# CX9898/sddmm-gpu

Measured on AMD Instinct MI355X. Metric: SDDMM GFLOP/s (2·nnz·K) + HBM GB/s %peak, K=128, 1/2/4/8 MI355X, higher is better.
Workload: dtype f32

## Files before the change

sddmm-gpu_amd/csrc/sddmm.hip:

```cpp
#include <algorithm>
#include <type_traits>
#include <cmath>
#include <vector>

#include "common.hpp"
#include "plan.hpp"

namespace bsmr {
namespace {

typedef float f32x4 __attribute__((ext_vector_type(4)));

struct SddmmArgs {
    const float* A;
    const float* B;
    float* P;
    u32 d0, nd;
    const u32* tileRows;
    const u32* rows;
    u32 R, N, K;
    const u32* denseCols;
    const u32* blockValues;
    const uint2* slots;
    u32 nslots;
// ... 302 lines not shown
}

struct RbArgs {
    const char* A;
    const char* B;
    float* P;
    const u32* rows;
    u32 R, N, RB;
    u32 qbase;
    u32 row0;
    const uint4* items;
    const u32* itemEnd;
    const uint2* pieces;
    const u32* meta;
    const u32* out;
    const uint4* tilePanel;
    const u32* tileIds;
    const u32* denseCols;
    const u32* blockValues;
    u32 mode;
    u32 outLds;
    u32 outPacked;
    u32 stageNt;
    u32 lateB;
    u32 stageBlocks;
    const u32* sortedPos;
    const uint2* itemEnt;
    const uint2* runs;
    const uint2* itemRuns;
    u32 pairs;
    unsigned long long* trace;
    u32 diag;
    unsigned long long bA, bB, bP;
};

typedef float f32x2 __attribute__((ext_vector_type(2)));
typedef _Float16 h16x2 __attribute__((ext_vector_type(2)));
typedef __bf16 b16x2 __attribute__((ext_vector_type(2)));
typedef _Float16 h16x8 __attribute__((ext_vector_type(8)));
typedef __bf16 b16x8 __attribute__((ext_vector_type(8)));

template <int DT>
__device__ __forceinline__ u32 lds_chunk(u32 lr, u32 c) {
    if constexpr (DT == 0)
        return c;
    else
        return (c & ~3u) | ((c & 3u) ^ (lr & 3u));
}

__device__ __forceinline__ f32x4 ld16(const char* p) { return *reinterpret_cast<const f32x4*>(p); }

__device__ __forceinline__ u32 lds_addr(const char* l) {
    return __builtin_amdgcn_readfirstlane(static_cast<u32>(
        reinterpret_cast<uintptr_t>((__attribute__((address_space(3))) const char*)l)));
}
template <int AUX>
__device__ __forceinline__ void rb_dma16(const char* g, const u32 m0) {
    if constexpr (AUX == 2)
        asm volatile("s_mov_b32 m0, %1\n\ts_nop 0\n\tglobal_load_lds_dwordx4 %0, off nt" ::"v"(g), "s"(m0)
                     : "memory", "m0");
    else
        asm volatile("s_mov_b32 m0, %1\n\ts_nop 0\n\tglobal_load_lds_dwordx4 %0, off" ::"v"(g), "s"(m0)
                     : "memory", "m0");
}

template <int I>
__device__ __forceinline__ u32 quad_bcast(u32 v) {
    return static_cast<u32>(
        __builtin_amdgcn_update_dpp(0, static_cast<int>(v), I * 0x55, 0xF, 0xF, false));
}

template <int DT>
__device__ __forceinline__ void chunk_dot(const f32x4 a, const f32x4 b, f32x2& acc0, f32x2& acc1) {
    if constexpr (DT == 0) {
        acc0 = __builtin_elementwise_fma(f32x2{a.x, a.y}, f32x2{b.x, b.y}, acc0);
        acc1 = __builtin_elementwise_fma(f32x2{a.z, a.w}, f32x2{b.z, b.w}, acc1);
    } else if constexpr (DT == 1) {
        const h16x8 ha = __builtin_bit_cast(h16x8, a), hb = __builtin_bit_cast(h16x8, b);
        acc0.x = __builtin_amdgcn_fdot2(ha.s01, hb.s01, acc0.x, false);
        acc0.y = __builtin_amdgcn_fdot2(ha.s23, hb.s23, acc0.y, false);
        acc1.x = __builtin_amdgcn_fdot2(ha.s45, hb.s45, acc1.x, false);
        acc1.y = __builtin_amdgcn_fdot2(ha.s67, hb.s67, acc1.y, false);
    } else {
        const b16x8 ha = __builtin_bit_cast(b16x8, a), hb = __builtin_bit_cast(b16x8, b);
        acc0.x = __builtin_amdgcn_fdot2_f32_bf16(ha.s01, hb.s01, acc0.x, false);
        acc0.y = __builtin_amdgcn_fdot2_f32_bf16(ha.s23, hb.s23, acc0.y, false);
        acc1.x = __builtin_amdgcn_fdot2_f32_bf16(ha.s45, hb.s45, acc1.x, false);
        acc1.y = __builtin_amdgcn_fdot2_f32_bf16(ha.s67, hb.s67, acc1.y, false);
    }
}

template <int DT>
__device__ __forceinline__ f32x4 chunk_mfma(const f32x4 a, const f32x4 b, f32x4 acc) {
    if constexpr (DT == 0) {
        acc = __builtin_amdgcn_mfma_f32_16x16x4f32(a.x, b.x, acc, 0, 0, 0);
        acc = __builtin_amdgcn_mfma_f32_16x16x4f32(a.y, b.y, acc, 0, 0, 0);
        acc = __builtin_amdgcn_mfma_f32_16x16x4f32(a.z, b.z, acc, 0, 0, 0);
        return __builtin_amdgcn_mfma_f32_16x16x4f32(a.w, b.w, acc, 0, 0, 0);
    } else if constexpr (DT == 1) {
        return __builtin_amdgcn_mfma_f32_16x16x32_f16(__builtin_bit_cast(h16x8, a),
                                                      __builtin_bit_cast(h16x8, b), acc, 0, 0, 0);
    } else {
        return __builtin_amdgcn_mfma_f32_16x16x32_bf16(__builtin_bit_cast(b16x8, a),
                                                       __builtin_bit_cast(b16x8, b), acc, 0, 0, 0);
    }
}

template <int RBY>
struct RowGeom {
    static constexpr u32 G = RBY >= 2048 ? 16 : RBY >= 1024 ? 8 : 4;
    static constexpr u32 NC = RBY / (16 * G);
    static constexpr u32 NB = (RB_PIECE_MAX + G - 1) / G;
    static constexpr u32 RR = (G == 4 ? 4u : G == 8 ? 2u : 1u) < NC ? (G == 4 ? 4u : G == 8 ? 2u : 1u) : NC;
};

template <int G, int I>
__device__ __forceinline__ u32 group_bcast(u32 v) {
    if constexpr (G == 4)
        return quad_bcast<I>(v);
    else if constexpr (G == 8)
        return static_cast<u32>(__builtin_amdgcn_ds_swizzle(static_cast<int>(v), 0x18 | (I << 5)));
    else
        return row_bcast<I>(v);
}

template <int DT, int RBY>
struct DenseTileLds {
    static constexpr int NK = RBY / 64;
    static constexpr int CH = NK > 8 ? 8 : NK;
    u32 lr, c, idx[4];
    __device__ __forceinline__ static u32 chunk(int kk, u32 g) {
        if constexpr (NK >= 4)
            return 16 * (kk >> 2) + 4 * g + (kk & 3);
        else
            return NK * g + kk;
    }
    __device__ __forceinline__ void meta(const RbArgs& a, const u32 tile, const u32 q0) {
        const u32 l = __lane_id(), rr = l & 15, g = l >> 4;
        const u32 p = a.tilePanel[tile].x;
        c = a.denseCols[tile * 16 + rr];
        const u32* bvals = a.blockValues + static_cast<size_t>(tile) * 256 + 64 * g + rr;
#pragma unroll
        for (int r = 0; r < 4; ++r) idx[r] = bvals[16 * r];
        lr = p * 16 - q0 + rr;
    }
    __device__ __forceinline__ void loadB(const RbArgs& a, const int k0, f32x4 (&bv)[CH]) const {
        const u32 g = __lane_id() >> 4;
        const bool cvalid = c < a.N;
        const char* bcol = a.B + static_cast<size_t>(cvalid && !(a.diag & 8388608u) ? c : 0) * RBY;
#pragma unroll
        for (int kk = 0; kk < CH; ++kk)
            bv[kk] = cvalid ? ld16(bcol + 16 * chunk(k0 + kk, g)) : f32x4{0, 0, 0, 0};
    }
    __device__ __forceinline__ void load(const RbArgs& a, const u32 tile, const u32 q0,
                                         f32x4 (&bv)[CH]) {
        meta(a, tile, q0);
        loadB(a, 0, bv);
    }
    __device__ __forceinline__ void run(const RbArgs& a, const char* As, f32x4 (&bv)[CH]) const {
        const u32 g = __lane_id() >> 4;
        const char* arow = As + lr * RBY;
        f32x4 acc0 = {0, 0, 0, 0}, acc1 = {0, 0, 0, 0};
#pragma unroll
        for (int k0 = 0; k0 < NK; k0 += CH) {
            if (k0) loadB(a, k0, bv);
#pragma unroll
            for (int kk = 0; kk < CH; ++kk) {
                const f32x4 av = ld16(arow + 16 * lds_chunk<DT>(lr, chunk(k0 + kk, g)));
                f32x4& acc = (kk & 1) ? acc1 : acc0;
                acc = chunk_mfma<DT>(av, bv[kk], acc);
            }
        }
        const f32x4 acc = acc0 + acc1;
#pragma unroll
        for (int r = 0; r < 4; ++r)
            if (idx[r] != NULLV) a.P[idx[r]] = acc[r];
    }
};

template <int RBY>
__device__ __forceinline__ void load_bcol(const RbArgs& a, const u32 col, const u32 sub,
                                          const u32 (&rot)[RowGeom<RBY>::NC],
                                          f32x4 (&bv)[RowGeom<RBY>::NC]) {
    const u32 bb = ((a.diag & 64) ? 0u : col) * RBY + 16 * sub;
#pragma unroll
    for (u32 f = 0; f < RowGeom<RBY>::NC; ++f)
        bv[f] = f + RowGeom<RBY>::RR <= RowGeom<RBY>::NC
                    ? ld16(a.B + (bb + rot[0]) + 16 * RowGeom<RBY>::G * f)
                    : ld16(a.B + (bb + rot[f]));
}

template <int RBY>
struct Piece {
    u32 first, len, col;
    u32 mm[RowGeom<RBY>::NB], mo[RowGeom<RBY>::NB];
};

template <int RBY>
__device__ __forceinline__ void load_piece_desc(const RbArgs& a, const u32 pi, Piece<RBY>& pc) {
    const uint2 d = a.pieces[pi];
    pc.first = d.x;
    pc.len = (d.y >> 22) + 1;
    pc.col = d.y & 0x3FFFFFu;
}

template <int RBY>
__device__ __forceinline__ void load_piece_body(const RbArgs& a, const u32 sub,
                                                const u32 (&rot)[RowGeom<RBY>::NC],
                                                f32x4 (&bv)[RowGeom<RBY>::NC], Piece<RBY>& pc) {
    constexpr u32 G = RowGeom<RBY>::G;
    load_bcol<RBY>(a, pc.col, sub, rot, bv);
#pragma unroll
    for (u32 k = 0; k < RowGeom<RBY>::NB; ++k) {
        const u32 e = G * k + sub;
        pc.mm[k] = e < pc.len ? a.meta[pc.first + e] : 0u;
        pc.mo[k] = !a.outLds && !a.outPacked && e < pc.len ? a.out[pc.first + e] : 0u;
    }
}

template <int RBY>
__device__ __forceinline__ void load_piece(const RbArgs& a, const u32 pi, const u32 sub,
                                           const u32 (&rot)[RowGeom<RBY>::NC],
                                           f32x4 (&bv)[RowGeom<RBY>::NC], Piece<RBY>& pc) {
    load_piece_desc<RBY>(a, pi, pc);
    load_piece_body<RBY>(a, sub, rot, bv, pc);
}

template <int DT, int RBY>
__device__ __forceinline__ void residual_piece(const RbArgs& a, const char* As,
                                               const Piece<RBY>& pc, const u32 sub,
                                               const u32 (&rot)[RowGeom<RBY>::NC],
                                               const f32x4 (&bv)[RowGeom<RBY>::NC]) {
    constexpr u32 G = RowGeom<RBY>::G, NC = RowGeom<RBY>::NC;
#pragma unroll
    for (u32 k = 0; k < RowGeom<RBY>::NB; ++k) {
        if (G * k >= pc.len) break;
        const u32 nb = min(G, pc.len - G * k);
        const u32 mk = DT == 0 ? (pc.mm[k] >> 22) * RBY : pc.mm[k];
        float res = 0.f;
#pragma unroll
        for (int i = 0; i < static_cast<int>(G); ++i) {
            if (static_cast<u32>(i) >= nb) break;
            u32 m;
            switch (i) {
#define BSMR_C(I) \
    case I: m = group_bcast<G, (I < G ? I : 0)>(mk); break;
                BSMR_C(0) BSMR_C(1) BSMR_C(2) BSMR_C(3) BSMR_C(4) BSMR_C(5) BSMR_C(6) BSMR_C(7)
                BSMR_C(8) BSMR_C(9) BSMR_C(10) BSMR_C(11) BSMR_C(12) BSMR_C(13) BSMR_C(14)
#undef BSMR_C
                default: m = group_bcast<G, G - 1>(mk); break;
            }
            u32 ab;
            if constexpr (DT == 0) {
                ab = m + 16 * sub;
            } else {
                const u32 lr = m >> 22;
                ab = lr * RBY + 16 * lds_chunk<DT>(lr, sub);
            }
            const char* arot = As + (ab + rot[0]);
            f32x2 acc0 = {0.f, 0.f}, acc1 = {0.f, 0.f};
            constexpr u32 H = NC > 4 ? NC / 2 : NC;
#pragma unroll
            for (u32 h = 0; h < NC; h += H) {
                f32x4 av[H];
#pragma unroll
                for (u32 f = 0; f < H; ++f)
                    av[f] = h + f + RowGeom<RBY>::RR <= NC ? ld16(arot + 16 * G * (h + f))
                                                           : ld16(As + (ab + rot[h + f]));
#pragma unroll
                for (u32 f = 0; f < H; ++f) {
                    if constexpr (DT == 0)
                        chunk_dot<DT>(av[f], bv[h + f], acc0, acc0);
                    else
                        chunk_dot<DT>(av[f], bv[h + f], acc0, acc1);
                }
            }
            f32x2 acc = acc0;
            if constexpr (DT != 0) acc += acc1;
            float sm = acc.x + acc.y;
            sm += dppf<0xB1>(sm);
            sm += dppf<0x4E>(sm);
            if constexpr (G >= 8) sm += dppf<0x141>(sm);
            if constexpr (G == 16) sm += dppf<0x140>(sm);
            if (sub == static_cast<u32>(i)) res = sm;
        }
        if (sub < nb) {
            if (a.outLds)
                *reinterpret_cast<float*>(const_cast<char*>(As) + a.outLds +
                                          4 * (pc.mm[k] & 0x3FFFFFu)) = res;
            else
                a.P[a.outPacked ? pc.mm[k] & 0x3FFFFFu : pc.mo[k]] = res;
        }
    }
}

constexpr u32 BATCH_CTR_BYTES = 16;
template <int DT, int RBY, int NT, typename LoadRuns>
__device__ __forceinline__ void rb_batches(const RbArgs& a, const char* As, const u32 p0, const u32 np,
                                           const u32 gr, const u32 sub, const u32 (&rot)[RowGeom<RBY>::NC],
                                           Piece<RBY>& pc, f32x4 (&pre)[RowGeom<RBY>::NC], LoadRuns&& load_runs) {
    constexpr u32 NC = RowGeom<RBY>::NC, GW = 64 / RowGeom<RBY>::G, NW = NT / 64;
    u32* const ctr = reinterpret_cast<u32*>(const_cast<char*>(As) + (NT == 1024 ? 160u : 80u) * 1024u - 4u);
    auto grab = [&]() -> u32 {
        u32 v = 0;
        if ((threadIdx.x & 63) == 0)
            v = __hip_atomic_fetch_add(ctr, 1u, __ATOMIC_RELAXED, __HIP_MEMORY_SCOPE_WORKGROUP);
        return NW + static_cast<u32>(__builtin_amdgcn_readfirstlane(static_cast<int>(v)));
    };
    Piece<RBY> pn;
    f32x4 nb[NC];
    auto fetch = [&](const u32 b) {
        const u32 pi = b * GW + gr % GW;
        pn.len = 0;
        if (pi < np) load_piece<RBY>(a, p0 + pi, sub, rot, nb, pn);
    };
    u32 bn = grab();
    if (bn * GW < np)
        fetch(bn);
    else
        load_runs();
    if (pc.len) residual_piece<DT, RBY>(a, As, pc, sub, rot, pre);
    while (bn * GW < np) {
        pc = pn;
#pragma unroll
        for (u32 f = 0; f < NC; ++f) pre[f] = nb[f];
        bn = grab();
        if (bn * GW < np)
            fetch(bn);
        else
            load_runs();
        if (pc.len) residual_piece<DT, RBY>(a, As, pc, sub, rot, pre);
    }
}

constexpr u32 NO_ITEM = 0xFFFFFFFFu;
constexpr u32 PAIR_RUNS_PER_WAVE = 16;

template <int RBY, int NT>
__device__ __forceinline__ u32 rb_stage_rows(const RbArgs& a, const u32 q0, const u32 ws, const u32 lane) {
    constexpr u32 NW = NT / 64, NCH = RBY / 16, NR = NCH >= 64 ? 1 : 64 / NCH;
    constexpr u32 MAXB = (NT == 1024 ? 160u : 80u) / NW;
    const u32 i = lane / NR, b = ws + i * NW, lr = 64 * b / NCH + lane % NR, q = q0 + lr;
    return (i < MAXB && lr < a.RB && q < a.R) ? a.rows[q] : a.row0;
}

template <int DT, int RBY, int NT, int AUX>
__device__ __forceinline__ void rb_stage_issue(const RbArgs& a, char* As, u32 rowv, const u32 ws,
                                               const u32 lane) {
    constexpr u32 NW = NT / 64, NCH = RBY / 16, NR = NCH >= 64 ? 1 : 64 / NCH;
    asm volatile("" : "+v"(rowv));
    constexpr u32 MAXB = (NT == 1024 ? 160u : 80u) / NW;
    const u32 x0 = 64 * ws + lane;
    const u32 coff = 16 * lds_chunk<DT>(x0 / NCH, x0 % NCH);
#pragma unroll 2
    for (u32 i = 0; i < MAXB; ++i) {
        const u32 b = ws + i * NW;
        u32 src = static_cast<u32>(__builtin_amdgcn_readlane(static_cast<int>(rowv), i * NR));
#pragma unroll
        for (u32 k = 1; k < NR; ++k) {
            const u32 rk = static_cast<u32>(__builtin_amdgcn_readlane(static_cast<int>(rowv), i * NR + k));
            src = lane / NCH == k ? rk : src;
        }
        const char* g = a.A + (static_cast<size_t>(src) * RBY + coff);
        if (b < a.stageBlocks) rb_dma16<AUX>(g, lds_addr(As) + 1024 * b);
    }
}

template <int DT, int RBY, int NT, int OM, bool DYN = false>
__device__ __forceinline__ bool rb_item(const RbArgs& a, char* As, const u32 idx, const bool prestaged,
                                        const u32 next) {
    constexpr bool PAIR = OM == 2, STAGED = OM != 0, LEAN = OM >= 2;
    using Geo = RowGeom<RBY>;
    constexpr u32 G = Geo::G, NC = Geo::NC;
    constexpr u32 NW = NT / 64;
    constexpr u32 NG = NT / G;
    constexpr u32 TC = DenseTileLds<DT, RBY>::CH;
    const unsigned long long t0 = LEAN ? 0ull : rtime(a.trace);
    uint4 it = a.items[idx];
    it.x = __builtin_amdgcn_readfirstlane(it.x);
    it.y = __builtin_amdgcn_readfirstlane(it.y);
    it.z = __builtin_amdgcn_readfirstlane(it.z);
    it.w = __builtin_amdgcn_readfirstlane(it.w);
    const u32 pend = a.itemEnd[idx];
    if (it.y == it.z && it.w == pend) return false;
    bool has_next = false, same_rb = false;
    u32 q0n = 0;
    if (next != NO_ITEM) {
        uint4 nt = a.items[next];
        nt.x = __builtin_amdgcn_readfirstlane(nt.x);
        nt.y = __builtin_amdgcn_readfirstlane(nt.y);
        nt.z = __builtin_amdgcn_readfirstlane(nt.z);
        nt.w = __builtin_amdgcn_readfirstlane(nt.w);
        const u32 nend = __builtin_amdgcn_readfirstlane(a.itemEnd[next]);
        has_next = !(nt.y == nt.z && nt.w == nend);
        q0n = a.qbase + nt.x * a.RB;
        same_rb = nt.x == it.x;
    }
    const u32 q0 = a.qbase + it.x * a.RB;
    u32 tid = threadIdx.x;
    if constexpr (LEAN) asm volatile("" : "+v"(tid));
    const u32 w = tid >> 6, sub = tid % G, j = (tid & 63) / G;
    const u32 ntile = !LEAN && (a.mode & 1) ? it.z - it.y : 0u;
    const u32 np = (a.mode & 2) ? pend - it.w : 0u;
    const u32 gr = tid / G;
    u32 rot[NC];
#pragma unroll
    for (u32 f = 0; f < NC; ++f) rot[f] = 16u * G * ((f + j % Geo::RR) % NC);
    constexpr u32 NCH = RBY / 16;
    constexpr u32 NR = NCH >= 64 ? 1 : 64 / NCH;
    constexpr u32 MAXB = (NT == 1024 ? 160u : 80u) / NW;
    static_assert(MAXB * NW == (NT == 1024 ? 160u : 80u), "whole KiB blocks");
    constexpr bool ROWV = MAXB * NR <= 64;
    const u32 lane = tid & 63;
    const u32 ws = __builtin_amdgcn_readfirstlane(w);
    u32 rowv = 0;
    u32 src[ROWV ? 1 : MAXB];
    if (!prestaged) {
        if constexpr (ROWV) {
            rowv = rb_stage_rows<RBY, NT>(a, q0, ws, lane);
        } else {
#pragma unroll
            for (u32 i = 0; i < MAXB; ++i) {
                const u32 lr = 64 * (ws + i * NW) / NCH + lane / NCH, q = q0 + lr;
                src[i] = lr < a.RB && q < a.R ? a.rows[q] : a.row0;
            }
#pragma unroll
            for (u32 i = 0; i < MAXB; ++i) asm volatile("" : "+v"(src[i]));
        }
    }
    f32x4 tb[TC], pre[NC];
    DenseTileLds<DT, RBY> dt;
    const u32 tw = NW - 1 - w;
    Piece<RBY> pc;
    pc.len = 0;
    if constexpr (!LEAN)
        if (tw < ntile) dt.meta(a, a.tileIds[it.y + tw], q0);
    if (gr < np) load_piece_desc<RBY>(a, it.w + gr, pc);
    uint2 myrun = make_uint2(0u, 0u), irun = make_uint2(0u, 0u);
    u32 rown = a.row0;
    auto load_runs = [&]() {
        if (STAGED && a.runs && a.outLds) {
            irun = a.itemRuns[idx];
            irun.x = __builtin_amdgcn_readfirstlane(irun.x);
            irun.y = __builtin_amdgcn_readfirstlane(irun.y);
            const u32 jr = w + NW * lane;
            if (jr < irun.y) myrun = a.runs[irun.x + jr];
        }
        if constexpr (ROWV)
            if (has_next && !same_rb) rown = rb_stage_rows<RBY, NT>(a, q0n, ws, lane);
    };
    auto stage = [&](auto aux_tag) {
        constexpr int AUX = decltype(aux_tag)::value;
        if constexpr (ROWV) {
            rb_stage_issue<DT, RBY, NT, AUX>(a, As, rowv, ws, lane);
        } else {
            const u32 x0 = 64 * ws + lane;
            const u32 coff = 16 * lds_chunk<DT>(x0 / NCH, x0 % NCH);
#pragma unroll
            for (u32 i = 0; i < MAXB; ++i) {
                const u32 b = ws + i * NW;
                const char* g = a.A + (static_cast<size_t>(src[i]) * RBY + coff);
                if (b < a.stageBlocks) rb_dma16<AUX>(g, lds_addr(As) + 1024 * b);
            }
        }
    };
    if (!prestaged) {
        if (!LEAN && a.stageNt)
            stage(std::integral_constant<int, 2>{});
        else
            stage(std::integral_constant<int, 0>{});
    }
    if (!LEAN && !a.lateB) {
        if (gr < np) load_piece_body<RBY>(a, sub, rot, pre, pc);
        if (tw < ntile) dt.loadB(a, 0, tb);
    }
    if constexpr (DYN)
        if (tid == 0) *reinterpret_cast<u32*>(As + (NT == 1024 ? 160u : 80u) * 1024u - 4u) = 0u;
    asm volatile("s_waitcnt vmcnt(0)" ::: "memory");
    __syncthreads();
    if (LEAN || a.lateB) {
        if (gr < np) load_piece_body<RBY>(a, sub, rot, pre, pc);
        if constexpr (!LEAN)
            if (tw < ntile) dt.loadB(a, 0, tb);
    }
    const unsigned long long tm = LEAN ? 0ull : rtime(a.trace);
    if (!LEAN && (a.diag & 8)) {
        trace_wave(a.trace, idx * NW + w, t0, tm);
        return false;
    }
    if constexpr (!LEAN)
        if (tw < ntile) dt.run(a, As, tb);
    const unsigned long long td = LEAN ? 0ull : rtime(a.trace);
    if constexpr (DYN) {
        rb_batches<DT, RBY, NT>(a, As, it.w, np, gr, sub, rot, pc, pre, [] {});
    } else {
        Piece<RBY> pn;
        f32x4 nb[NC];
        auto fetch = [&](const u32 ph) {
            const u32 pi = ph * NG + ((ph & 1) ? NG - 1 - gr : gr);
            pn.len = 0;
            if (pi < np) load_piece<RBY>(a, it.w + pi, sub, rot, nb, pn);
        };
        if (NG < np) fetch(1);
        if (pc.len) residual_piece<DT, RBY>(a, As, pc, sub, rot, pre);
        for (u32 ph = 1; ph * NG < np; ++ph) {
            pc = pn;
#pragma unroll
            for (u32 f = 0; f < NC; ++f) pre[f] = nb[f];
            if ((ph + 1) * NG < np) fetch(ph + 1);
            if (pc.len) residual_piece<DT, RBY>(a, As, pc, sub, rot, pre);
        }
    }
    if constexpr (STAGED) load_runs();
    if constexpr (!LEAN) {
        for (u32 t = it.y + tw + NW; t < it.z; t += NW) {
            dt.load(a, a.tileIds[t], q0, tb);
            dt.run(a, As, tb);
        }
    }
    bool staged_next = false;
    if (STAGED && a.outLds) {
        __syncthreads();
        const uint2 ie = a.itemEnt[idx];
        const float* res = reinterpret_cast<const float*>(As + a.outLds);
        const u32 nr = irun.y > w ? (irun.y - w + NW - 1) / NW : 0u;
        if constexpr (PAIR && ROWV) {
            if (has_next && __builtin_amdgcn_readfirstlane(irun.y) <= NW * PAIR_RUNS_PER_WAVE) {
                float v[PAIR_RUNS_PER_WAVE];
#pragma unroll
                for (u32 u = 0; u < PAIR_RUNS_PER_WAVE; ++u) {
                    const u32 sl = static_cast<u32>(__builtin_amdgcn_readlane(static_cast<int>(myrun.y), u));
                    const u32 len = u < nr ? sl >> 16 : 0u;
                    v[u] = lane < len ? res[(sl & 0xFFFFu) + lane] : 0.0f;
                }
                __syncthreads();
                rowv = rown;
                if (!same_rb) stage(std::integral_constant<int, 0>{});
#pragma unroll
                for (u32 u = 0; u < PAIR_RUNS_PER_WAVE; ++u) {
                    const u32 pos = static_cast<u32>(__builtin_amdgcn_readlane(static_cast<int>(myrun.x), u));
                    const u32 sl = static_cast<u32>(__builtin_amdgcn_readlane(static_cast<int>(myrun.y), u));
                    const u32 len = u < nr ? sl >> 16 : 0u;
                    if (lane < len) a.P[pos + lane] = v[u];
                }
                return true;
            }
        }
        if (LEAN || !(a.diag & 128)) {
            if (LEAN || a.runs) {
                for (u32 i = 0; i < nr; i += 4) {
                    u32 pos[4], s0[4], len[4];
                    float v[4];
#pragma unroll
                    for (u32 u = 0; u < 4; ++u) {
                        const u32 q = min(i + u, 63u);
                        pos[u] = static_cast<u32>(__builtin_amdgcn_readlane(static_cast<int>(myrun.x), q));
                        const u32 sl = static_cast<u32>(__builtin_amdgcn_readlane(static_cast<int>(myrun.y), q));
                        s0[u] = sl & 0xFFFFu;
                        len[u] = i + u < nr ? sl >> 16 : 0u;
                        v[u] = lane < len[u] ? res[s0[u] + lane] : 0.0f;
                    }
#pragma unroll
                    for (u32 u = 0; u < 4; ++u)
                        if (lane < len[u]) a.P[pos[u] + lane] = v[u];
                }
            } else if constexpr (!LEAN) {
                constexpr u32 U = 8;
                for (u32 t0s = tid; t0s < ie.y; t0s += U * NT) {
                    u32 pos[U];
#pragma unroll
                    for (u32 k = 0; k < U; ++k) {
                        const u32 t = t0s + k * NT;
                        pos[k] = t < ie.y ? a.sortedPos[ie.x + t] : 0u;
                    }
#pragma unroll
                    for (u32 k = 0; k < U; ++k) {
                        const u32 t = t0s + k * NT;
                        if (t < ie.y) a.P[pos[k]] = res[t];
                    }
                }
            }
        }
        if constexpr (PAIR && ROWV) {
            if (has_next) {
                __syncthreads();
                rowv = rown;
                if (!same_rb) stage(std::integral_constant<int, 0>{});
                staged_next = true;
            }
        }
    }
    if constexpr (!LEAN) trace_wave(a.trace, idx * NW + w, t0, tm, td);
    return staged_next;
}

template <int DT, int RBY, int NT, bool DYN, bool LITE = false>
__global__ __launch_bounds__(NT, 4) void k_sddmm_rb(RbArgs a) {
    extern __shared__ __attribute__((aligned(16))) char AsB[];
    char* As = AsB;
    if (blockIdx.y) {
        a.A += blockIdx.y * a.bA;
        a.B += blockIdx.y * a.bB;
        a.P += blockIdx.y * a.bP;
    }
    using Geo = RowGeom<RBY>;
    constexpr u32 G = Geo::G, NC = Geo::NC;
    constexpr u32 NW = NT / 64;
    constexpr u32 NG = NT / G;
    constexpr u32 TC = DenseTileLds<DT, RBY>::CH;
    const unsigned long long t0 = LITE ? 0ull : rtime(a.trace);
    uint4 it = a.items[blockIdx.x];
    it.x = __builtin_amdgcn_readfirstlane(it.x);
    it.y = __builtin_amdgcn_readfirstlane(it.y);
    it.z = __builtin_amdgcn_readfirstlane(it.z);
    it.w = __builtin_amdgcn_readfirstlane(it.w);
    const u32 pend = a.itemEnd[blockIdx.x];
    if (it.y == it.z && it.w == pend) return;
    const u32 q0 = a.qbase + it.x * a.RB;
    const u32 tid = threadIdx.x, w = tid >> 6, sub = tid % G, j = (tid & 63) / G;
    const u32 ntile = !LITE && (a.mode & 1) ? it.z - it.y : 0u;
    const u32 np = LITE || (a.mode & 2) ? pend - it.w : 0u;
    const u32 gr = tid / G;
    u32 rot[NC];
#pragma unroll
    for (u32 f = 0; f < NC; ++f) rot[f] = 16u * G * ((f + j % Geo::RR) % NC);
    constexpr u32 NCH = RBY / 16;
    constexpr u32 NR = NCH >= 64 ? 1 : 64 / NCH;
    constexpr u32 MAXB = (NT == 1024 ? 160u : 80u) / NW;
    static_assert(MAXB * NW == (NT == 1024 ? 160u : 80u), "whole KiB blocks");
    constexpr bool ROWV = MAXB * NR <= 64;
    const u32 lane = tid & 63;
    const u32 ws = __builtin_amdgcn_readfirstlane(w);
    u32 rowv = a.row0;
    u32 src[ROWV ? 1 : MAXB];
    if constexpr (ROWV) {
        const u32 i = lane / NR, b = ws + i * NW, lr = 64 * b / NCH + lane % NR, q = q0 + lr;
        if (i < MAXB && lr < a.RB && q < a.R) rowv = a.rows[q];
    } else {
#pragma unroll
        for (u32 i = 0; i < MAXB; ++i) {
            const u32 lr = 64 * (ws + i * NW) / NCH + lane / NCH, q = q0 + lr;
            src[i] = lr < a.RB && q < a.R ? a.rows[q] : a.row0;
        }
#pragma unroll
        for (u32 i = 0; i < MAXB; ++i) asm volatile("" : "+v"(src[i]));
    }
    f32x4 tb[TC], pre[NC];
    DenseTileLds<DT, RBY> dt;
    const u32 tw = NW - 1 - w;
    Piece<RBY> pc;
    pc.len = 0;
    if constexpr (!LITE)
        if (tw < ntile) dt.meta(a, a.tileIds[it.y + tw], q0);
    if (gr < np) load_piece_desc<RBY>(a, it.w + gr, pc);
    uint2 myrun = make_uint2(0u, 0u), irun = make_uint2(0u, 0u);
    auto load_runs = [&]() {
        if (!LITE && a.runs && a.outLds) {
            irun = a.itemRuns[blockIdx.x];
            irun.x = __builtin_amdgcn_readfirstlane(irun.x);
            irun.y = __builtin_amdgcn_readfirstlane(irun.y);
            const u32 j = w + NW * lane;
            if (j < irun.y) myrun = a.runs[irun.x + j];
        }
    };
    auto stage = [&](auto aux_tag) {
        constexpr int AUX = decltype(aux_tag)::value;
        const u32 x0 = 64 * ws + lane;
        const u32 coff = 16 * lds_chunk<DT>(x0 / NCH, x0 % NCH);
        if constexpr (ROWV) {
#pragma unroll
            for (u32 i = 0; i < MAXB; ++i) {
                const u32 b = ws + i * NW;
                u32 src = static_cast<u32>(__builtin_amdgcn_readlane(static_cast<int>(rowv), i * NR));
#pragma unroll
                for (u32 k = 1; k < NR; ++k) {
                    const u32 rk = static_cast<u32>(__builtin_amdgcn_readlane(static_cast<int>(rowv), i * NR + k));
                    src = lane / NCH == k ? rk : src;
                }
                const char* g = a.A + (static_cast<size_t>(src) * RBY + coff);
                if (b < a.stageBlocks) rb_dma16<AUX>(g, lds_addr(As) + 1024 * b);
            }
        } else {
#pragma unroll
            for (u32 i = 0; i < MAXB; ++i) {
                const u32 b = ws + i * NW;
                const char* g = a.A + (static_cast<size_t>(src[i]) * RBY + coff);
                if (b < a.stageBlocks) rb_dma16<AUX>(g, lds_addr(As) + 1024 * b);
            }
        }
    };
    if (!LITE && a.stageNt)
        stage(std::integral_constant<int, 2>{});
    else
        stage(std::integral_constant<int, 0>{});
    if (!LITE && !a.lateB) {
        if (gr < np) load_piece_body<RBY>(a, sub, rot, pre, pc);
        if (tw < ntile) dt.loadB(a, 0, tb);
    }
    if constexpr (DYN)
        if (tid == 0) *reinterpret_cast<u32*>(As + (NT == 1024 ? 160u : 80u) * 1024u - 4u) = 0u;
    asm volatile("s_waitcnt vmcnt(0)" ::: "memory");
    __syncthreads();
    if (LITE || a.lateB) {
        if (gr < np) load_piece_body<RBY>(a, sub, rot, pre, pc);
        if constexpr (!LITE)
            if (tw < ntile) dt.loadB(a, 0, tb);
    }
    const unsigned long long tm = LITE ? 0ull : rtime(a.trace);
    if (!LITE && (a.diag & 8)) {
        trace_wave(a.trace, blockIdx.x * NW + w, t0, tm);
        return;
    }
    if constexpr (!LITE)
        if (tw < ntile) dt.run(a, As, tb);
    const unsigned long long td = LITE ? 0ull : rtime(a.trace);
    if constexpr (DYN) {
        rb_batches<DT, RBY, NT>(a, As, it.w, np, gr, sub, rot, pc, pre, load_runs);
    } else {
        Piece<RBY> pn;
        f32x4 nb[NC];
        auto fetch = [&](const u32 ph) {
            const u32 pi = ph * NG + ((ph & 1) ? NG - 1 - gr : gr);
            pn.len = 0;
            if (pi < np) load_piece<RBY>(a, it.w + pi, sub, rot, nb, pn);
        };
        if (NG < np)
            fetch(1);
        else
            load_runs();
        if (pc.len) residual_piece<DT, RBY>(a, As, pc, sub, rot, pre);
        for (u32 ph = 1; ph * NG < np; ++ph) {
            pc = pn;
#pragma unroll
            for (u32 f = 0; f < NC; ++f) pre[f] = nb[f];
            if ((ph + 1) * NG < np)
                fetch(ph + 1);
            else
                load_runs();
            if (pc.len) residual_piece<DT, RBY>(a, As, pc, sub, rot, pre);
        }
    }
    if constexpr (LITE) return;
    for (u32 t = it.y + tw + NW; t < it.z; t += NW) {
        dt.load(a, a.tileIds[t], q0, tb);
        dt.run(a, As, tb);
    }
    if (a.outLds) {
        __syncthreads();
        const uint2 ie = a.itemEnt[blockIdx.x];
        const float* res = reinterpret_cast<const float*>(As + a.outLds);
        if (!(a.diag & 128)) {
            constexpr u32 U = 8;
            auto pass = [&]() {
                for (u32 t0 = tid; t0 < ie.y; t0 += U * NT) {
                    u32 pos[U];
#pragma unroll
                    for (u32 k = 0; k < U; ++k) {
                        const u32 t = t0 + k * NT;
                        pos[k] = t < ie.y ? a.sortedPos[ie.x + t] : 0u;
                    }
#pragma unroll
                    for (u32 k = 0; k < U; ++k) {
                        const u32 t = t0 + k * NT;
                        if (t < ie.y) a.P[pos[k]] = res[t];
                    }
                }
            };
            if (a.runs) {
                const u32 nr = irun.y > w ? (irun.y - w + NW - 1) / NW : 0u;
                for (u32 i = 0; i < nr; i += 4) {
                    u32 pos[4], s0[4], len[4];
                    float v[4];
#pragma unroll
                    for (u32 u = 0; u < 4; ++u) {
                        const u32 q = min(i + u, 63u);
                        pos[u] = static_cast<u32>(__builtin_amdgcn_readlane(static_cast<int>(myrun.x), q));
                        const u32 sl = static_cast<u32>(__builtin_amdgcn_readlane(static_cast<int>(myrun.y), q));
                        s0[u] = sl & 0xFFFFu;
                        len[u] = i + u < nr ? sl >> 16 : 0u;
                        v[u] = lane < len[u] ? res[s0[u] + lane] : 0.0f;
                    }
#pragma unroll
                    for (u32 u = 0; u < 4; ++u)
                        if (lane < len[u]) a.P[pos[u] + lane] = v[u];
                }
            } else {
                pass();
            }
        }
    }
    trace_wave(a.trace, blockIdx.x * NW + w, t0, tm, td);
}

template <int DT, int RBY, int NT, bool DYN>
__global__ __launch_bounds__(NT, 4) void k_sddmm_rb_pair(RbArgs a) {
    extern __shared__ __attribute__((aligned(16))) char AsB[];
    char* As = AsB;
    if (blockIdx.y) {
        a.A += blockIdx.y * a.bA;
        a.B += blockIdx.y * a.bB;
        a.P += blockIdx.y * a.bP;
    }
    const u32 x = blockIdx.x % XCD_BUCKETS, i0 = (blockIdx.x / XCD_BUCKETS) * 2 * XCD_BUCKETS + x;
    if (rb_item<DT, RBY, NT, 2, DYN>(a, As, i0, false, i0 + XCD_BUCKETS))
        rb_item<DT, RBY, NT, 2, DYN>(a, As, i0 + XCD_BUCKETS, true, NO_ITEM);
}

template <int DT, int RBY>
void (*pick_rb(const u32 NT, const bool pairs, const bool dyn, const bool lite))(RbArgs) {
    if constexpr (RBY >= 256) {
        if (pairs) {
            if constexpr (RBY <= 512)
                if (dyn) return NT == 1024 ? k_sddmm_rb_pair<DT, RBY, 1024, true> : k_sddmm_rb_pair<DT, RBY, 512, true>;
            return NT == 1024 ? k_sddmm_rb_pair<DT, RBY, 1024, false> : k_sddmm_rb_pair<DT, RBY, 512, false>;
        }
    }
    if constexpr (RBY <= 512)
        if (dyn) {
            if (lite) return NT == 1024 ? k_sddmm_rb<DT, RBY, 1024, true, true> : k_sddmm_rb<DT, RBY, 512, true, true>;
            return NT == 1024 ? k_sddmm_rb<DT, RBY, 1024, true> : k_sddmm_rb<DT, RBY, 512, true>;
        }
    if (lite) return NT == 1024 ? k_sddmm_rb<DT, RBY, 1024, false, true> : k_sddmm_rb<DT, RBY, 512, false, true>;
    return NT == 1024 ? k_sddmm_rb<DT, RBY, 1024, false> : k_sddmm_rb<DT, RBY, 512, false>;
}

static_assert(TILES_PER_ITEM == 1, "dense work items are single tiles (tile id = item id)");

using KernelFn = void (*)(SddmmArgs);

template <int G, bool PANELS>
KernelFn pick_k(u32 K) {
#define BSMR_K(KT) (PANELS ? k_sddmm_panels_f32<KT, G> : k_sddmm_f32<KT, G>)
    switch (K) {
        case 32: return BSMR_K(32);
        case 64: return BSMR_K(64);
        case 128: return BSMR_K(128);
        case 256: return BSMR_K(256);
        case 512: return BSMR_K(512);
        default: return BSMR_K(0);
    }
#undef BSMR_K
}

template <bool PANELS>
KernelFn pick_kernel(u32 K) {
    if (K % 64 == 0) return pick_k<16, PANELS>(K);
    if (K % 32 == 0) return pick_k<8, PANELS>(K);
    return pick_k<4, PANELS>(K);
}

int validate(const void* dA, const void* dB, u32 K, int dtype, const float* dP) {
    if (!dA || !dB || !dP) {
        set_error("bsmr_sddmm: null device pointer");
        return BSMR_ERR_INVALID;
    }
    return report(validate_kd("bsmr_sddmm", K, dtype));
}

SddmmArgs make_args(const Plan& p, const void* dA, const void* dB, u32 K, float* dP) {
    SddmmArgs a{};
    a.A = static_cast<const float*>(dA);
    a.B = static_cast<const float*>(dB);
    a.P = dP;
    a.tileRows = p.tileRows.data();
    a.rows = p.rows.data();
    a.R = p.R;
    a.N = p.N;
    a.K = K;
    a.denseCols = p.denseCols.data();
    a.blockValues = p.blockValues.data();
    a.slots = p.cmSlots.data();
    a.cmRow = p.cmRow.data();
    a.cmCol = p.cmCol.data();
    a.cmOut = p.cmOut.data();
    a.ritems = p.resItems.data();
    a.sparseValues = p.sparseValues.data();
    a.sparseRel = p.sparseRel.data();
    a.sparseCol = p.sparseColIdx.data();
    a.diag = p.diag;
    return a;
}

int get_rb_layout(const Plan& p, int slot, int dtype, u32 pa, u32 pb,
                  std::shared_ptr<const Plan::RowBlockLayout>* out, const LaunchSite* at = nullptr,
                  bool keep = false) {
    std::lock_guard<std::mutex> g(p.layout_mu);
    const u32 rowBytes = 128u << slot;
    const bool half = dtype != BSMR_F32;
    if (!keep) {
        *out = p.rowblock_ready(rowBytes, half, pa, pb);
        if (*out) return BSMR_OK;
        if (at) BSMR_CHECK(lazy_build_guard(*at));
    }
    int err = BSMR_OK;
// ... 462 lines not shown
```

Measured before the change: 20600.

## Software-pipeline piece descriptor loads two stages ahead with branchless clamped fetches

Restructures the residual-piece loop so descriptors are prefetched two iterations ahead (d1/d2), while bodies (meta, out, B columns) are loaded one ahead. Per-lane conditional loads are replaced by clamped index loads, and loop trip counts become wave-uniform via a per-wave activity check. This is meant to hide the dependent descriptor-to-body load latency and remove divergent branches. In exchange it issues redundant clamped loads for inactive lanes and adds register pressure from the extra in-flight descriptors.

Result: faster. 21060 (median of 6 runs) (+2.2%).

```diff
diff --git a/sddmm-gpu_amd/csrc/sddmm.hip b/sddmm-gpu_amd/csrc/sddmm.hip
--- a/sddmm-gpu_amd/csrc/sddmm.hip
+++ b/sddmm-gpu_amd/csrc/sddmm.hip
@@ -522,34 +522,30 @@
     u32 mm[RowGeom<RBY>::NB], mo[RowGeom<RBY>::NB];
 };
 
+
+__device__ __forceinline__ uint2 load_piece_desc(const RbArgs& a, const u32 p0, const u32 np, const u32 pi) {
+    return a.pieces[p0 + min(pi, np - 1u)];
+}
+
 template <int RBY>
-__device__ __forceinline__ void load_piece_desc(const RbArgs& a, const u32 pi, Piece<RBY>& pc) {
-    const uint2 d = a.pieces[pi];
-    pc.first = d.x;
-    pc.len = (d.y >> 22) + 1;
-    pc.col = d.y & 0x3FFFFFu;
-}
-
-template <int RBY>
-__device__ __forceinline__ void load_piece_body(const RbArgs& a, const u32 sub,
+__device__ __forceinline__ void load_piece_body(const RbArgs& a, const uint2 d, const bool has,
+                                                const bool use_out, const u32 sub,
                                                 const u32 (&rot)[RowGeom<RBY>::NC],
                                                 f32x4 (&bv)[RowGeom<RBY>::NC], Piece<RBY>& pc) {
-    constexpr u32 G = RowGeom<RBY>::G;
+    constexpr u32 G = RowGeom<RBY>::G, NB = RowGeom<RBY>::NB;
+    const u32 last = d.y >> 22;
+    pc.first = d.x;
+    pc.len = has ? last + 1u : 0u;
+    pc.col = d.y & 0x3FFFFFu;
+#pragma unroll
+    for (u32 k = 0; k < NB; ++k) pc.mo[k] = 0u;
+    if (use_out) {
+#pragma unroll
+        for (u32 k = 0; k < NB; ++k) pc.mo[k] = a.out[d.x + min(G * k + sub, last)];
+    }
     load_bcol<RBY>(a, pc.col, sub, rot, bv);
 #pragma unroll
-    for (u32 k = 0; k < RowGeom<RBY>::NB; ++k) {
-        const u32 e = G * k + sub;
-        pc.mm[k] = e < pc.len ? a.meta[pc.first + e] : 0u;
-        pc.mo[k] = !a.outLds && !a.outPacked && e < pc.len ? a.out[pc.first + e] : 0u;
-    }
-}
-
-template <int RBY>
-__device__ __forceinline__ void load_piece(const RbArgs& a, const u32 pi, const u32 sub,
-                                           const u32 (&rot)[RowGeom<RBY>::NC],
-                                           f32x4 (&bv)[RowGeom<RBY>::NC], Piece<RBY>& pc) {
-    load_piece_desc<RBY>(a, pi, pc);
-    load_piece_body<RBY>(a, sub, rot, bv, pc);
+    for (u32 k = 0; k < NB; ++k) pc.mm[k] = a.meta[d.x + min(G * k + sub, last)];
 }
 
 template <int DT, int RBY>
@@ -624,7 +620,8 @@
 template <int DT, int RBY, int NT, typename LoadRuns>
 __device__ __forceinline__ void rb_batches(const RbArgs& a, const char* As, const u32 p0, const u32 np,
                                            const u32 gr, const u32 sub, const u32 (&rot)[RowGeom<RBY>::NC],
-                                           Piece<RBY>& pc, f32x4 (&pre)[RowGeom<RBY>::NC], LoadRuns&& load_runs) {
+                                           Piece<RBY>& pc, f32x4 (&pre)[RowGeom<RBY>::NC], const bool use_out,
+                                           LoadRuns&& load_runs) {
     constexpr u32 NC = RowGeom<RBY>::NC, GW = 64 / RowGeom<RBY>::G, NW = NT / 64;
     u32* const ctr = reinterpret_cast<u32*>(const_cast<char*>(As) + (NT == 1024 ? 160u : 80u) * 1024u - 4u);
     auto grab = [&]() -> u32 {
@@ -633,30 +630,47 @@
             v = __hip_atomic_fetch_add(ctr, 1u, __ATOMIC_RELAXED, __HIP_MEMORY_SCOPE_WORKGROUP);
         return NW + static_cast<u32>(__builtin_amdgcn_readfirstlane(static_cast<int>(v)));
     };
-    Piece<RBY> pn;
-    f32x4 nb[NC];
-    auto fetch = [&](const u32 b) {
-        const u32 pi = b * GW + gr % GW;
-        pn.len = 0;
-        if (pi < np) load_piece<RBY>(a, p0 + pi, sub, rot, nb, pn);
-    };
-    u32 bn = grab();
-    if (bn * GW < np)
-        fetch(bn);
-    else
-        load_runs();
+    u32 b1 = grab();
+    uint2 d1 = load_piece_desc(a, p0, np, b1 * GW + gr % GW);
+    while (b1 * GW < np) {
+        const u32 b2 = grab();
+        const uint2 d2 = load_piece_desc(a, p0, np, b2 * GW + gr % GW);
+        Piece<RBY> pn;
+        f32x4 nb[NC];
+        load_piece_body<RBY>(a, d1, b1 * GW + gr % GW < np, use_out, sub, rot, nb, pn);
+        if (pc.len) residual_piece<DT, RBY>(a, As, pc, sub, rot, pre);
+        pc = pn;
+#pragma unroll
+        for (u32 f = 0; f < NC; ++f) pre[f] = nb[f];
+        d1 = d2;
+        b1 = b2;
+    }
+    load_runs();
     if (pc.len) residual_piece<DT, RBY>(a, As, pc, sub, rot, pre);
-    while (bn * GW < np) {
+}
+
+template <int DT, int RBY, int NT, typename LoadRuns>
+__device__ __forceinline__ void rb_phases(const RbArgs& a, const char* As, const u32 p0, const u32 np,
+                                          const u32 gr, const u32 ws, const u32 sub,
+                                          const u32 (&rot)[RowGeom<RBY>::NC], Piece<RBY>& pc,
+                                          f32x4 (&pre)[RowGeom<RBY>::NC], uint2 d1, const bool use_out,
+                                          LoadRuns&& load_runs) {
+    constexpr u32 NC = RowGeom<RBY>::NC, GW = 64 / RowGeom<RBY>::G, NG = NT / RowGeom<RBY>::G;
+    auto piece_of = [&](const u32 ph) { return ph * NG + ((ph & 1) ? NG - 1 - gr : gr); };
+    auto wave_first = [&](const u32 ph) { return ph * NG + ((ph & 1) ? NG - (ws + 1) * GW : ws * GW); };
+    for (u32 ph = 0; wave_first(ph + 1) < np; ++ph) {
+        const uint2 d2 = load_piece_desc(a, p0, np, piece_of(ph + 2));
+        Piece<RBY> pn;
+        f32x4 nb[NC];
+        load_piece_body<RBY>(a, d1, piece_of(ph + 1) < np, use_out, sub, rot, nb, pn);
+        if (pc.len) residual_piece<DT, RBY>(a, As, pc, sub, rot, pre);
         pc = pn;
 #pragma unroll
         for (u32 f = 0; f < NC; ++f) pre[f] = nb[f];
-        bn = grab();
-        if (bn * GW < np)
-            fetch(bn);
-        else
-            load_runs();
-        if (pc.len) residual_piece<DT, RBY>(a, As, pc, sub, rot, pre);
-    }
+        d1 = d2;
+    }
+    load_runs();
+    if (pc.len) residual_piece<DT, RBY>(a, As, pc, sub, rot, pre);
 }
 
 constexpr u32 NO_ITEM = 0xFFFFFFFFu;
@@ -761,7 +775,16 @@
     pc.len = 0;
     if constexpr (!LEAN)
         if (tw < ntile) dt.meta(a, a.tileIds[it.y + tw], q0);
-    if (gr < np) load_piece_desc<RBY>(a, it.w + gr, pc);
+    constexpr u32 GW = 64 / G;
+    const bool wact = ws * GW < np;
+    const bool use_out = !PAIR && !a.outLds && !a.outPacked;
+    uint2 d0 = make_uint2(0u, 0u), d1 = make_uint2(0u, 0u);
+    if (wact) {
+        d0 = load_piece_desc(a, it.w, np, gr);
+        if constexpr (!DYN) d1 = load_piece_desc(a, it.w, np, 2 * NG - 1 - gr);
+        asm volatile("" : "+v"(d0.x), "+v"(d0.y), "+v"(d1.x), "+v"(d1.y));
+    }
+    auto body0 = [&]() { load_piece_body<RBY>(a, d0, gr < np, use_out, sub, rot, pre, pc); };
     uint2 myrun = make_uint2(0u, 0u), irun = make_uint2(0u, 0u);
     u32 rown = a.row0;
     auto load_runs = [&]() {
@@ -797,7 +820,7 @@
             stage(std::integral_constant<int, 0>{});
     }
     if (!LEAN && !a.lateB) {
-        if (gr < np) load_piece_body<RBY>(a, sub, rot, pre, pc);
+        if (wact) body0();
         if (tw < ntile) dt.loadB(a, 0, tb);
     }
     if constexpr (DYN)
@@ -805,7 +828,7 @@
     asm volatile("s_waitcnt vmcnt(0)" ::: "memory");
     __syncthreads();
     if (LEAN || a.lateB) {
-        if (gr < np) load_piece_body<RBY>(a, sub, rot, pre, pc);
+        if (wact) body0();
         if constexpr (!LEAN)
             if (tw < ntile) dt.loadB(a, 0, tb);
     }
@@ -817,25 +840,11 @@
     if constexpr (!LEAN)
         if (tw < ntile) dt.run(a, As, tb);
     const unsigned long long td = LEAN ? 0ull : rtime(a.trace);
-    if constexpr (DYN) {
-        rb_batches<DT, RBY, NT>(a, As, it.w, np, gr, sub, rot, pc, pre, [] {});
-    } else {
-        Piece<RBY> pn;
-        f32x4 nb[NC];
-        auto fetch = [&](const u32 ph) {
-            const u32 pi = ph * NG + ((ph & 1) ? NG - 1 - gr : gr);
-            pn.len = 0;
-            if (pi < np) load_piece<RBY>(a, it.w + pi, sub, rot, nb, pn);
-        };
-        if (NG < np) fetch(1);
-        if (pc.len) residual_piece<DT, RBY>(a, As, pc, sub, rot, pre);
-        for (u32 ph = 1; ph * NG < np; ++ph) {
-            pc = pn;
-#pragma unroll
-            for (u32 f = 0; f < NC; ++f) pre[f] = nb[f];
-            if ((ph + 1) * NG < np) fetch(ph + 1);
-            if (pc.len) residual_piece<DT, RBY>(a, As, pc, sub, rot, pre);
-        }
+    if (wact) {
+        if constexpr (DYN)
+            rb_batches<DT, RBY, NT>(a, As, it.w, np, gr, sub, rot, pc, pre, use_out, [] {});
+        else
+            rb_phases<DT, RBY, NT>(a, As, it.w, np, gr, ws, sub, rot, pc, pre, d1, use_out, [] {});
     }
     if constexpr (STAGED) load_runs();
     if constexpr (!LEAN) {
@@ -978,7 +987,16 @@
     pc.len = 0;
     if constexpr (!LITE)
         if (tw < ntile) dt.meta(a, a.tileIds[it.y + tw], q0);
-    if (gr < np) load_piece_desc<RBY>(a, it.w + gr, pc);
+    constexpr u32 GW = 64 / G;
+    const bool wact = ws * GW < np;
+    const bool use_out = !a.outLds && !a.outPacked;
+    uint2 d0 = make_uint2(0u, 0u), d1 = make_uint2(0u, 0u);
+    if (wact) {
+        d0 = load_piece_desc(a, it.w, np, gr);
+        if constexpr (!DYN) d1 = load_piece_desc(a, it.w, np, 2 * NG - 1 - gr);
+        asm volatile("" : "+v"(d0.x), "+v"(d0.y), "+v"(d1.x), "+v"(d1.y));
+    }
+    auto body0 = [&]() { load_piece_body<RBY>(a, d0, gr < np, use_out, sub, rot, pre, pc); };
     uint2 myrun = make_uint2(0u, 0u), irun = make_uint2(0u, 0u);
     auto load_runs = [&]() {
         if (!LITE && a.runs && a.outLds) {
@@ -1020,7 +1038,7 @@
     else
         stage(std::integral_constant<int, 0>{});
     if (!LITE && !a.lateB) {
-        if (gr < np) load_piece_body<RBY>(a, sub, rot, pre, pc);
+        if (wact) body0();
         if (tw < ntile) dt.loadB(a, 0, tb);
     }
     if constexpr (DYN)
@@ -1028,7 +1046,7 @@
     asm volatile("s_waitcnt vmcnt(0)" ::: "memory");
     __syncthreads();
     if (LITE || a.lateB) {
-        if (gr < np) load_piece_body<RBY>(a, sub, rot, pre, pc);
+        if (wact) body0();
         if constexpr (!LITE)
             if (tw < ntile) dt.loadB(a, 0, tb);
     }
@@ -1040,32 +1058,12 @@
     if constexpr (!LITE)
         if (tw < ntile) dt.run(a, As, tb);
     const unsigned long long td = LITE ? 0ull : rtime(a.trace);
-    if constexpr (DYN) {
-        rb_batches<DT, RBY, NT>(a, As, it.w, np, gr, sub, rot, pc, pre, load_runs);
-    } else {
-        Piece<RBY> pn;
-        f32x4 nb[NC];
-        auto fetch = [&](const u32 ph) {
-            const u32 pi = ph * NG + ((ph & 1) ? NG - 1 - gr : gr);
-            pn.len = 0;
-            if (pi < np) load_piece<RBY>(a, it.w + pi, sub, rot, nb, pn);
-        };
-        if (NG < np)
-            fetch(1);
-        else
-            load_runs();
-        if (pc.len) residual_piece<DT, RBY>(a, As, pc, sub, rot, pre);
-        for (u32 ph = 1; ph * NG < np; ++ph) {
-            pc = pn;
-#pragma unroll
-            for (u32 f = 0; f < NC; ++f) pre[f] = nb[f];
-            if ((ph + 1) * NG < np)
-                fetch(ph + 1);
-            else
-                load_runs();
-            if (pc.len) residual_piece<DT, RBY>(a, As, pc, sub, rot, pre);
-        }
-    }
+    if (!wact)
+        load_runs();
+    else if constexpr (DYN)
+        rb_batches<DT, RBY, NT>(a, As, it.w, np, gr, sub, rot, pc, pre, use_out, load_runs);
+    else
+        rb_phases<DT, RBY, NT>(a, As, it.w, np, gr, ws, sub, rot, pc, pre, d1, use_out, load_runs);
     if constexpr (LITE) return;
     for (u32 t = it.y + tw + NW; t < it.z; t += NW) {
         dt.load(a, a.tileIds[t], q0, tb);
```

## Issue residual piece and dense-tile B loads alongside A staging before barrier

Applied to the files above, without the earlier changes.

When early B loading is selected, the kernel now issues the piece metadata loads, the A-row LDS staging DMA, and the residual and dense-tile B column loads together, then waits only on the staging DMA with a partial vmcnt before the barrier. Previously B loads were serialized either before a full vmcnt(0) wait or after the barrier. Invalid dense-tile columns are loaded from a clamped address and zeroed afterward. Descriptor loads are made branch-free with clamped indices. The LITE path keeps the old behavior because the new flag is off. The change relies on the order of vmcnt counting matching the issue order; a miscount would be a correctness risk.

Result: slower. 22050 before, 21710 after (-1.5%).

```diff
diff --git a/sddmm-gpu_amd/csrc/sddmm.hip b/sddmm-gpu_amd/csrc/sddmm.hip
--- a/sddmm-gpu_amd/csrc/sddmm.hip
+++ b/sddmm-gpu_amd/csrc/sddmm.hip
@@ -478,6 +478,18 @@
         for (int kk = 0; kk < CH; ++kk)
             bv[kk] = cvalid ? ld16(bcol + 16 * chunk(k0 + kk, g)) : f32x4{0, 0, 0, 0};
     }
+    __device__ __forceinline__ void loadB_all(const RbArgs& a, f32x4 (&bv)[CH]) const {
+        const u32 g = __lane_id() >> 4;
+        const char* bcol = a.B + static_cast<size_t>(c < a.N && !(a.diag & 8388608u) ? c : 0) * RBY;
+#pragma unroll
+        for (int kk = 0; kk < CH; ++kk) bv[kk] = ld16(bcol + 16 * chunk(kk, g));
+    }
+    __device__ __forceinline__ void clearB(const RbArgs& a, f32x4 (&bv)[CH]) const {
+        if (!(c < a.N)) {
+#pragma unroll
+            for (int kk = 0; kk < CH; ++kk) bv[kk] = f32x4{0, 0, 0, 0};
+        }
+    }
     __device__ __forceinline__ void load(const RbArgs& a, const u32 tile, const u32 q0,
                                          f32x4 (&bv)[CH]) {
         meta(a, tile, q0);
@@ -531,17 +543,22 @@
 }
 
 template <int RBY>
-__device__ __forceinline__ void load_piece_body(const RbArgs& a, const u32 sub,
-                                                const u32 (&rot)[RowGeom<RBY>::NC],
-                                                f32x4 (&bv)[RowGeom<RBY>::NC], Piece<RBY>& pc) {
+__device__ __forceinline__ void load_piece_meta(const RbArgs& a, const u32 sub, Piece<RBY>& pc) {
     constexpr u32 G = RowGeom<RBY>::G;
-    load_bcol<RBY>(a, pc.col, sub, rot, bv);
 #pragma unroll
     for (u32 k = 0; k < RowGeom<RBY>::NB; ++k) {
         const u32 e = G * k + sub;
         pc.mm[k] = e < pc.len ? a.meta[pc.first + e] : 0u;
         pc.mo[k] = !a.outLds && !a.outPacked && e < pc.len ? a.out[pc.first + e] : 0u;
     }
+}
+
+template <int RBY>
+__device__ __forceinline__ void load_piece_body(const RbArgs& a, const u32 sub,
+                                                const u32 (&rot)[RowGeom<RBY>::NC],
+                                                f32x4 (&bv)[RowGeom<RBY>::NC], Piece<RBY>& pc) {
+    load_bcol<RBY>(a, pc.col, sub, rot, bv);
+    load_piece_meta<RBY>(a, sub, pc);
 }
 
 template <int RBY>
@@ -920,6 +937,8 @@
     return staged_next;
 }
 
+constexpr bool LEAN_EARLY_B = false;
+
 template <int DT, int RBY, int NT, bool DYN, bool LITE = false>
 __global__ __launch_bounds__(NT, 4) void k_sddmm_rb(RbArgs a) {
     extern __shared__ __attribute__((aligned(16))) char AsB[];
@@ -974,11 +993,29 @@
     f32x4 tb[TC], pre[NC];
     DenseTileLds<DT, RBY> dt;
     const u32 tw = NW - 1 - w;
-    Piece<RBY> pc;
+    Piece<RBY> pc, pn;
     pc.len = 0;
+    pn.len = 0;
+    dt.c = 0;
     if constexpr (!LITE)
         if (tw < ntile) dt.meta(a, a.tileIds[it.y + tw], q0);
-    if (gr < np) load_piece_desc<RBY>(a, it.w + gr, pc);
+    const bool early = LITE ? LEAN_EARLY_B : !a.lateB;
+    constexpr bool PH1 = LITE && LEAN_EARLY_B && !DYN;
+    if (early) {
+        pc.first = pn.first = 0;
+        pc.col = pn.col = 0;
+        if (np) {
+            load_piece_desc<RBY>(a, it.w + (gr < np ? gr : 0u), pc);
+            if (gr >= np) pc.len = 0;
+            if constexpr (PH1) {
+                const u32 p1 = 2 * NG - 1 - gr;
+                load_piece_desc<RBY>(a, it.w + (p1 < np ? p1 : 0u), pn);
+                if (p1 >= np) pn.len = 0;
+            }
+        }
+    } else if (gr < np) {
+        load_piece_desc<RBY>(a, it.w + gr, pc);
+    }
     uint2 myrun = make_uint2(0u, 0u), irun = make_uint2(0u, 0u);
     auto load_runs = [&]() {
         if (!LITE && a.runs && a.outLds) {
@@ -1015,19 +1052,34 @@
             }
         }
     };
-    if (!LITE && a.stageNt)
-        stage(std::integral_constant<int, 2>{});
-    else
-        stage(std::integral_constant<int, 0>{});
-    if (!LITE && !a.lateB) {
-        if (gr < np) load_piece_body<RBY>(a, sub, rot, pre, pc);
-        if (tw < ntile) dt.loadB(a, 0, tb);
-    }
+    auto stage_item = [&]() {
+        if (!LITE && a.stageNt)
+            stage(std::integral_constant<int, 2>{});
+        else
+            stage(std::integral_constant<int, 0>{});
+    };
     if constexpr (DYN)
         if (tid == 0) *reinterpret_cast<u32*>(As + (NT == 1024 ? 160u : 80u) * 1024u - 4u) = 0u;
-    asm volatile("s_waitcnt vmcnt(0)" ::: "memory");
-    __syncthreads();
-    if (LITE || a.lateB) {
+    if (early) {
+        if constexpr (ROWV) asm volatile("" : "+v"(rowv));
+        asm volatile("" : "+v"(pc.first), "+v"(pc.len), "+v"(pc.col));
+        if constexpr (PH1) asm volatile("" : "+v"(pn.first), "+v"(pn.len), "+v"(pn.col));
+        if constexpr (!LITE)
+            asm volatile("" : "+v"(dt.lr), "+v"(dt.c), "+v"(dt.idx[0]), "+v"(dt.idx[1]), "+v"(dt.idx[2]),
+                         "+v"(dt.idx[3]));
+        load_piece_meta<RBY>(a, sub, pc);
+        stage_item();
+        load_bcol<RBY>(a, pc.col, sub, rot, pre);
+        if constexpr (!LITE) dt.loadB_all(a, tb);
+        constexpr u32 NB0 = LITE ? NC : NC + TC;
+        asm volatile("s_waitcnt vmcnt(%0)" ::"n"(NB0) : "memory");
+        __syncthreads();
+        if constexpr (!LITE)
+            if (tw < ntile) dt.clearB(a, tb);
+    } else {
+        stage_item();
+        asm volatile("s_waitcnt vmcnt(0)" ::: "memory");
+        __syncthreads();
         if (gr < np) load_piece_body<RBY>(a, sub, rot, pre, pc);
         if constexpr (!LITE)
             if (tw < ntile) dt.loadB(a, 0, tb);
@@ -1043,17 +1095,21 @@
     if constexpr (DYN) {
         rb_batches<DT, RBY, NT>(a, As, it.w, np, gr, sub, rot, pc, pre, load_runs);
     } else {
-        Piece<RBY> pn;
         f32x4 nb[NC];
         auto fetch = [&](const u32 ph) {
             const u32 pi = ph * NG + ((ph & 1) ? NG - 1 - gr : gr);
             pn.len = 0;
             if (pi < np) load_piece<RBY>(a, it.w + pi, sub, rot, nb, pn);
         };
-        if (NG < np)
-            fetch(1);
-        else
+        if (NG < np) {
+            if constexpr (PH1) {
+                if (pn.len) load_piece_body<RBY>(a, sub, rot, nb, pn);
+            } else {
+                fetch(1);
+            }
+        } else {
             load_runs();
+        }
         if (pc.len) residual_piece<DT, RBY>(a, As, pc, sub, rot, pre);
         for (u32 ph = 1; ph * NG < np; ++ph) {
             pc = pn;
```
